# IanMadlenya/pyconsensus

Hardware: AMD Instinct MI355X
Metric: oracle rounds/sec (batched 50x20, 1 GPU) (higher is better)
Workload: dtype f64; 1 GPU; C3: 65536 independent 50x20 oracle rounds per GPU per step (one wavefront per round), inputs resident in HBM, every output of the result dict written (original and filled included); rounds_per_gpu=65536, reporters=50, events=20, parallelism=rounds sharded across 1 GPU(s), no collective

## Files before the change

### pyconsensus_amd/csrc/pcx_batched.hip

```cpp
#include <hip/hip_runtime.h>
#include <stdint.h>
#include <stdlib.h>

#include "pcx_internal.h"

namespace pcx {

namespace {

constexpr int W = 64;
constexpr int NMAX = 64;
constexpr int EMAX = 32;
static_assert(EMAX <= 2 * 16, "2 x 2 grid of 16 x 16 MFMA tiles");
static_assert(NMAX == W, "one reporter per lane");
constexpr int PACKED_WAVES = 4;

constexpr double PI_TOL = 1e-14;
constexpr int PI_MAXIT = 256;
constexpr int PI_PRESQUARE = 3;
constexpr int PI_SQUARE_EVERY = 32;
constexpr int PI_MAX_SQUARINGS = 8;
constexpr int PI_POLISH = 2;
constexpr double DBL_MIN_ = 2.2250738585072014e-308;
constexpr double DBL_EPS = 2.220446049250313080847e-16;

__device__ __forceinline__ int lane_id() { return threadIdx.x; }

#define PCX_OUTLINE __forceinline__

#define STAMP(k)                                                                  \
    do {                                                                          \
        if (a.stamps) {                                                           \
            const long long t_ = (long long)__builtin_amdgcn_s_memtime();         \
            if (threadIdx.x == 0) a.stamps[b * 32 + (k)] = t_;                    \
        }                                                                         \
    } while (0)

__device__ __forceinline__ void wsync() {
    __builtin_amdgcn_fence(__ATOMIC_RELEASE, "wavefront");
    __builtin_amdgcn_wave_barrier();
    __builtin_amdgcn_fence(__ATOMIC_ACQUIRE, "wavefront");
}

__device__ __forceinline__ uint64_t ballot(bool p) { return __ballot(p); }

__device__ __forceinline__ int popc(uint64_t m) { return __popcll(m); }

__device__ __forceinline__ double bcast(double v, int src) {
    const uint64_t u = (uint64_t)__double_as_longlong(v);
    const uint32_t lo = (uint32_t)__builtin_amdgcn_readlane((int)(uint32_t)u, src);
    const uint32_t hi = (uint32_t)__builtin_amdgcn_readlane((int)(uint32_t)(u >> 32), src);
    return __longlong_as_double((long long)(((uint64_t)hi << 32) | lo));
}

template <int CTRL>
__device__ __forceinline__ uint32_t dpp32(uint32_t v) {
    return (uint32_t)__builtin_amdgcn_update_dpp(0, (int)v, CTRL, 0xf, 0xf, false);
}
template <int S>
__device__ __forceinline__ uint32_t xor_lane32(uint32_t v) {
    if constexpr (S == 1) return dpp32<0xB1>(v);
    else if constexpr (S == 2) return dpp32<0x4E>(v);
    else if constexpr (S == 8) return dpp32<0x128>(v);
    else {
        static_assert(S == 4, "row-local distances only");
        const uint32_t up = dpp32<0x114>(v), dn = dpp32<0x104>(v);
        return (threadIdx.x & 4) ? up : dn;
    }
}

template <int S>
__device__ __forceinline__ double xor_lane(double v) {
    const uint64_t u = (uint64_t)__double_as_longlong(v);
    const uint32_t lo = xor_lane32<S>((uint32_t)u), hi = xor_lane32<S>((uint32_t)(u >> 32));
    return __longlong_as_double((long long)(((uint64_t)hi << 32) | lo));
}

__device__ __forceinline__ double lane_value(double v, int k) {
    const uint64_t u = (uint64_t)__double_as_longlong(v);
    const uint32_t lo = (uint32_t)__builtin_amdgcn_readlane((int)(uint32_t)u, k);
    const uint32_t hi = (uint32_t)__builtin_amdgcn_readlane((int)(uint32_t)(u >> 32), k);
    return __longlong_as_double((long long)(((uint64_t)hi << 32) | lo));
}

template <int ROWS = 4>
__device__ __forceinline__ double tree_sum(double v) {
    static_assert(ROWS == 1 || ROWS == 2 || ROWS == 4, "live 16-lane rows");
    v = v + xor_lane<1>(v);
    v = v + xor_lane<2>(v);
    v = v + xor_lane<4>(v);
    v = v + xor_lane<8>(v);
    if constexpr (ROWS == 1) return lane_value(v, 0);
    if constexpr (ROWS == 2) return lane_value(v, 0) + lane_value(v, 16);
    return (lane_value(v, 0) + lane_value(v, 16)) + (lane_value(v, 32) + lane_value(v, 48));
}
constexpr int live_rows(int ET) { return ET > 0 ? (ET <= 16 ? 1 : ET <= 32 ? 2 : 4) : 4; }

template <int D>
__device__ __forceinline__ double shr_lane(double v) {
    const uint64_t u = (uint64_t)__double_as_longlong(v);
    const uint32_t lo = (uint32_t)__builtin_amdgcn_update_dpp(0, (int)(uint32_t)u, 0x110 + D, 0xf, 0xf, false);
    const uint32_t hi = (uint32_t)__builtin_amdgcn_update_dpp(0, (int)(uint32_t)(u >> 32), 0x110 + D, 0xf, 0xf, false);
    return __longlong_as_double((long long)(((uint64_t)hi << 32) | lo));
}
__device__ __forceinline__ double wave_scan_d(double v) {
    v = v + shr_lane<1>(v);
    v = v + shr_lane<2>(v);
    v = v + shr_lane<4>(v);
    v = v + shr_lane<8>(v);
    const double r0 = lane_value(v, 15), r1 = lane_value(v, 31), r2 = lane_value(v, 47);
    const int row = threadIdx.x >> 4;
    const double r01 = r0 + r1;
    return row == 0 ? v : v + (row == 1 ? r0 : row == 2 ? r01 : r01 + r2);
}

template <int ROWS = 4>
__device__ __forceinline__ double wave_max(double v) {
    static_assert(ROWS == 1 || ROWS == 2 || ROWS == 4, "live 16-lane rows");
    v = fmax(v, xor_lane<1>(v));
    v = fmax(v, xor_lane<2>(v));
    v = fmax(v, xor_lane<4>(v));
    v = fmax(v, xor_lane<8>(v));
    if constexpr (ROWS == 1) return lane_value(v, 0);
    if constexpr (ROWS == 2) return fmax(lane_value(v, 0), lane_value(v, 16));
    return fmax(fmax(lane_value(v, 0), lane_value(v, 16)), fmax(lane_value(v, 32), lane_value(v, 48)));
}

__device__ __forceinline__ double catch_(double x, double tol) {
    if (x < 1.5 - tol) return 1.0;
    if (x > 1.5 + tol) return 2.0;
    return 1.5;
}

__device__ __forceinline__ double readlane_d(double v, int k) {
    const uint64_t u = (uint64_t)__double_as_longlong(v);
    const uint32_t lo = (uint32_t)__builtin_amdgcn_readlane((int)(uint32_t)u, k);
    const uint32_t hi = (uint32_t)__builtin_amdgcn_readlane((int)(uint32_t)(u >> 32), k);
    return __longlong_as_double((long long)(((uint64_t)hi << 32) | lo));
}

__device__ __forceinline__ double shr1_d(double v) {
    const uint64_t u = (uint64_t)__double_as_longlong(v);
    const uint32_t lo = (uint32_t)__builtin_amdgcn_update_dpp(0, (int)(uint32_t)u, 0x138, 0xf, 0xf, true);
    const uint32_t hi = (uint32_t)__builtin_amdgcn_update_dpp(0, (int)(uint32_t)(u >> 32), 0x138, 0xf, 0xf, true);
    return __longlong_as_double((long long)(((uint64_t)hi << 32) | lo));
}

__device__ __forceinline__ double permute_d(int dst_lane, double v) {
    const uint64_t u = (uint64_t)__double_as_longlong(v);
    const uint32_t lo = (uint32_t)__builtin_amdgcn_ds_permute(dst_lane * 4, (int)(uint32_t)u);
    const uint32_t hi = (uint32_t)__builtin_amdgcn_ds_permute(dst_lane * 4, (int)(uint32_t)(u >> 32));
    return __longlong_as_double((long long)(((uint64_t)hi << 32) | lo));
}

__device__ __forceinline__ double bpermute_d(int src_lane, double v) {
    const uint64_t u = (uint64_t)__double_as_longlong(v);
    const uint32_t lo = (uint32_t)__builtin_amdgcn_ds_bpermute(src_lane * 4, (int)(uint32_t)u);
    const uint32_t hi = (uint32_t)__builtin_amdgcn_ds_bpermute(src_lane * 4, (int)(uint32_t)(u >> 32));
    return __longlong_as_double((long long)(((uint64_t)hi << 32) | lo));
}

__device__ __forceinline__ int mbcnt64(uint64_t m) {
    return __builtin_amdgcn_mbcnt_hi((uint32_t)(m >> 32), __builtin_amdgcn_mbcnt_lo((uint32_t)m, 0));
}

__device__ PCX_OUTLINE double wave_pw_sum(double v, bool sel) {
    const int l = lane_id();
    const uint64_t m = ballot(sel);
    const int n = popc(m);
    if (n < 8) {
        double res = 0.0;
        uint64_t mm = m;
        while (mm) {
            const int k = __builtin_ctzll(mm);
            mm &= mm - 1;
            res += readlane_d(v, k);
        }
        return res;
    }
    const int p = sel ? mbcnt64(m) : n + mbcnt64(~m);
    const double a = permute_d((p & 7) * 8 + (p >> 3), v);
    const int T = n >> 3;
    double c = a;
    for (int t = 1; t < T; t++) {
        const double prev = shr1_d(c);
        c = (l & 7) == 0 ? a : prev + a;
    }
    const double r0 = readlane_d(c, 0 * 8 + T - 1), r1 = readlane_d(c, 1 * 8 + T - 1);
    const double r2 = readlane_d(c, 2 * 8 + T - 1), r3 = readlane_d(c, 3 * 8 + T - 1);
    const double r4 = readlane_d(c, 4 * 8 + T - 1), r5 = readlane_d(c, 5 * 8 + T - 1);
    const double r6 = readlane_d(c, 6 * 8 + T - 1), r7 = readlane_d(c, 7 * 8 + T - 1);
    double res = ((r0 + r1) + (r2 + r3)) + ((r4 + r5) + (r6 + r7));
    for (int q = 8 * T; q < n; q++) res += readlane_d(a, (q & 7) * 8 + (q >> 3));
    return res;
}

template <int NC>
__device__ PCX_OUTLINE double wave_pw_sum_prefix(double v, int nrt) {
    const int l = lane_id();
    const int n = NC > 0 ? NC : nrt;
    if (n < 8) {
        double res = 0.0;
        for (int k = 0; k < n; k++) res += readlane_d(v, k);
        return res;
    }
    const double a = permute_d((l & 7) * 8 + (l >> 3), v);
    const int T = n >> 3;
    double c = a;
    for (int t = 1; t < T; t++) {
        const double prev = shr1_d(c);
        c = (l & 7) == 0 ? a : prev + a;
    }
    const double r0 = readlane_d(c, 0 * 8 + T - 1), r1 = readlane_d(c, 1 * 8 + T - 1);
    const double r2 = readlane_d(c, 2 * 8 + T - 1), r3 = readlane_d(c, 3 * 8 + T - 1);
    const double r4 = readlane_d(c, 4 * 8 + T - 1), r5 = readlane_d(c, 5 * 8 + T - 1);
    const double r6 = readlane_d(c, 6 * 8 + T - 1), r7 = readlane_d(c, 7 * 8 + T - 1);
    double res = ((r0 + r1) + (r2 + r3)) + ((r4 + r5) + (r6 + r7));
    for (int q = 8 * T; q < n; q++) res += readlane_d(a, (q & 7) * 8 + (q >> 3));
    return res;
}

template <int D>
__device__ __forceinline__ double shl_lane(double v) {
    const uint64_t u = (uint64_t)__double_as_longlong(v);
    const uint32_t lo = dpp32<0x100 + D>((uint32_t)u), hi = dpp32<0x100 + D>((uint32_t)(u >> 32));
    return __longlong_as_double((long long)(((uint64_t)hi << 32) | lo));
}

__device__ __forceinline__ double pw_tree8(double c) {
    c = c + xor_lane<1>(c);
    c = c + xor_lane<2>(c);
    return c + shl_lane<4>(c);
}

template <int NC>
__device__ PCX_OUTLINE double wave_pw_sum_lds(double v, int nrt, double* scr) {
    const int l = lane_id();
    const int n = NC > 0 ? NC : nrt;
    if (n < 8) {
        double res = 0.0;
        for (int k = 0; k < n; k++) res += readlane_d(v, k);
        return res;
    }
    wsync();
    if (l < n) scr[l] = v;
    wsync();
    const int T = n >> 3;
    const double* const p = scr + (l & 7);
    double c = p[0];
    if constexpr (NC > 0) {
#pragma unroll
        for (int t = 1; t < NC / 8; t++) c = c + p[8 * t];
    } else {
        for (int t = 1; t < T; t++) c = c + p[8 * t];
    }
    c = pw_tree8(c);
    for (int q = 8 * T; q < n; q++) c = c + scr[q];
    return readlane_d(c, 0);
}

template <int NC>
__device__ PCX_OUTLINE void wave_pw_sum2_lds(double v1, double v2, int nrt, double* scr, double& s1, double& s2) {
    const int l = lane_id();
    const int n = NC > 0 ? NC : nrt;
    if (n < 8) {
        double r1 = 0.0, r2 = 0.0;
        for (int k = 0; k < n; k++) {
            r1 += readlane_d(v1, k);
            r2 += readlane_d(v2, k);
        }
        s1 = r1;
        s2 = r2;
        return;
    }
    wsync();
    if (l < n) {
        scr[l] = v1;
        scr[n + l] = v2;
    }
    wsync();
    const int T = n >> 3;
    const double* const base = scr + ((l & 8) ? n : 0);
    const double* const p = base + (l & 7);
    double c = p[0];
    if constexpr (NC > 0) {
#pragma unroll
        for (int t = 1; t < NC / 8; t++) c = c + p[8 * t];
    } else {
        for (int t = 1; t < T; t++) c = c + p[8 * t];
    }
    c = pw_tree8(c);
    for (int q = 8 * T; q < n; q++) c = c + base[q];
    s1 = readlane_d(c, 0);
    s2 = readlane_d(c, 8);
}

template <int NC>
__device__ PCX_OUTLINE double wave_pw_sum_dpp(double v, int nrt) {
    const int n = NC > 0 ? NC : nrt;
    if (n < 8 || n >= 24) return wave_pw_sum_prefix<NC>(v, nrt);
    const int T = n >> 3;
    double c = v;
    if (T == 2) c = v + shl_lane<8>(v);
    c = pw_tree8(c);
    double res = readlane_d(c, 0);
    for (int q = 8 * T; q < n; q++) res += readlane_d(v, q);
    return res;
}

__device__ __forceinline__ double dot2(const double* a, const double* b, int bs, int n) {
    double s = 0.0, c = 0.0;
    for (int i = 0; i < n; i++) {
        const double x = a[i], y = b[i * bs];
        const double p = x * y;
        const double pe = fma(x, y, -p);
        const double t = s + p;
        const double z = t - s;
        const double se = (s - (t - z)) + (p - z);
        s = t;
        c = c + (pe + se);
    }
    return s + c;
}

__device__ __noinline__ double ob_ddot(const double* v, const double* f, int ld, int n) {
    double acc8[4][8], acc4[4][4];
#pragma unroll
    for (int r = 0; r < 4; r++)
#pragma unroll
        for (int q = 0; q < 8; q++) acc8[r][q] = 0.0;
    const int n32 = n & -32, n16 = n & -16;
    for (int i = 0; i < n32; i += 32)
#pragma unroll
        for (int k = 0; k < 32; k++) acc8[k / 8][k % 8] = fma(v[i + k], f[(i + k) * ld], acc8[k / 8][k % 8]);
#pragma unroll
    for (int r = 0; r < 4; r++)
#pragma unroll
        for (int q = 0; q < 4; q++) acc4[r][q] = acc8[r][q] + acc8[r][q + 4];
    for (int i = n32; i < n16; i += 16)
#pragma unroll
        for (int k = 0; k < 16; k++) acc4[k / 4][k % 4] = fma(v[i + k], f[(i + k) * ld], acc4[k / 4][k % 4]);
    double A[4];
#pragma unroll
    for (int q = 0; q < 4; q++) A[q] = ((acc4[0][q] + acc4[1][q]) + acc4[2][q]) + acc4[3][q];
    double d = (A[0] + A[2]) + (A[1] + A[3]);
    for (int i = n16; i < n; i++) d = fma(v[i], f[i * ld], d);
    return d;
}

__device__ PCX_OUTLINE double ob_vecmat(const double* v, const double* f, int ld, int N, int E, int j) {
    if (E == 1) return ob_ddot(v, f, ld, N);
    if (j < (E & ~3)) {
        double y = 0.0;
        int n = 0;
        for (; n + 4 <= N; n += 4) {
            double t = f[(n + 1) * ld] * v[n + 1];
            t = fma(f[n * ld], v[n], t);
            t = fma(f[(n + 2) * ld], v[n + 2], t);
            t = fma(f[(n + 3) * ld], v[n + 3], t);
            y = y + t;
        }
        if (n + 2 <= N) {
            double t = f[(n + 1) * ld] * v[n + 1];
            t = fma(f[n * ld], v[n], t);
            y = y + t;
            n += 2;
        }
        if (n < N) y = y + f[n * ld] * v[n];
        return y;
    }
    double t = 0.0;
    int i = 0;
    if (E == 2 || E == 3)
        for (; i + 4 <= N; i += 4) {
            t = t + fma(f[i * ld], v[i], f[(i + 1) * ld] * v[i + 1]);
            t = t + fma(f[(i + 2) * ld], v[i + 2], f[(i + 3) * ld] * v[i + 3]);
        }
    for (; i < N; i++) t = fma(f[i * ld], v[i], t);
    return t;
// ... 274 lines not shown


__device__ __forceinline__ void round_to_global(double* dst, const double* F, int N, int E, int ES, int NT, int ET) {
    const int l = lane_id();
    if (NT > 0 && ET > 0 && (NT * ET) % 2 == 0 && ((uintptr_t)dst & 15) == 0) {
        const int tot2 = NT * ET / 2;
        for (int q = l; q < tot2; q += W) {
            const int idx = 2 * q;
            const int i0 = idx / ET, j0 = idx - i0 * ET;
            const int i1 = (idx + 1) / ET, j1 = idx + 1 - i1 * ET;
            reinterpret_cast<double2*>(dst)[q] = double2{F[i0 * ES + j0], F[i1 * ES + j1]};
        }
    } else {
        for (int idx = l; idx < N * E; idx += W) {
            const int i = idx / E, j = idx - i * E;
            dst[idx] = F[i * ES + j];
        }
    }
}

__device__ PCX_OUTLINE double rank_avg(const double* v, int E) {
    const int l = lane_id();
    double r = 0.0;
    if (l < E) {
        const double x = v[l];
        int lt = 0, eq = 0;
        for (int k = 0; k < E; k++) {
            const double y = v[k];
            lt += y < x;
            eq += y == x;
        }
        r = (double)lt + (double)(eq + 1) * 0.5;
        if (__builtin_isnan(x)) r = __builtin_nan("");
    }
    return r;
}

__device__ PCX_OUTLINE void rank_avg3(const double* v0, const double* v1, const double* v2, int E, double& r0,
                                      double& r1, double& r2) {
    const int l = lane_id();
    const int g = (l >= E) + (l >= 2 * E);
    const double* v = g == 0 ? v0 : g == 1 ? v1 : v2;
    double r = 0.0;
    if (l < 3 * E) {
        const double x = v[l - g * E];
        int lt = 0, eq = 0;
        for (int k = 0; k < E; k++) {
            const double y = v[k];
            lt += y < x;
            eq += y == x;
        }
        r = (double)lt + (double)(eq + 1) * 0.5;
        if (__builtin_isnan(x)) r = __builtin_nan("");
    }
    r0 = r;
    r1 = bpermute_d(l + E, r);
    r2 = bpermute_d(l + 2 * E, r);
}

struct Smem {
    double* F;
    double* C;
    double* M;
    double* rep;
    double* n1;
    double* n2;
    double* smooth;
    double* mu;
    double* tot;
    double* guess;
    double* x;
    double* ld;
    double* old;
    double* nv1;
    double* nv2;
    double* adj;
    uint64_t* miss;
};

__host__ __device__ inline int smem_rows(int N) { return (N + 1) & ~1; }
__host__ __device__ inline int cert_stride(int N, int ES) { return (ES & 1) ? (N | 1) : N; }
__host__ __device__ inline int smem_f_size(int N, int E, int ES) {
    return N * ES > E * cert_stride(N, ES) ? N * ES : E * cert_stride(N, ES);
}
__host__ __device__ inline int smem_evs(int E) { return (E + 1) & ~1; }
__host__ __device__ inline int smem_mat(int E, int ES, bool pk) { return pk ? E * (E + 1) / 2 : E * ES; }
__host__ __device__ inline int smem_c_size(int N, int E, int ES, bool pk) {
    if (pk) return smem_rows(N) + 2 * smem_evs(E);
    const int need = 3 * smem_rows(N) + 2 * smem_evs(E);
    return smem_mat(E, ES, pk) > need ? smem_mat(E, ES, pk) : need;
}
__host__ __device__ inline int smem_m_size(int N, int E, int ES, int NR, bool pk) {
    const int scr = med_scr(NR) + smem_evs(E);
    if (pk) {
        const int vec = 2 * smem_rows(N) + 2 * smem_evs(E);
        const int rest = smem_mat(E, ES, pk) - smem_c_size(N, E, ES, pk);
        const int need = scr > vec ? scr : vec;
        return need > rest ? need : rest;
    }
    const int need = scr > 2 * smem_evs(E) ? scr : 2 * smem_evs(E);
    return smem_mat(E, ES, pk) > need ? smem_mat(E, ES, pk) : need;
}

__host__ __device__ inline size_t smem_doubles(int N, int E, int ES, int NR, bool pk) {
    return (size_t)smem_f_size(N, E, ES) + smem_c_size(N, E, ES, pk) + smem_m_size(N, E, ES, NR, pk) +
           (pk ? 1 : 4) * (size_t)smem_evs(E);
}

template <bool PK>
__device__ __forceinline__ int sym_at(int j, int k, int ES) {
    if constexpr (PK)
        return j >= k ? j * (j + 1) / 2 + k : k * (k + 1) / 2 + j;
    else
        return j * ES + k;
}

__device__ Smem carve(double* base, int N, int E, int ES, int NR, bool pk) {
    const int nr = smem_rows(N), ne = smem_evs(E);
    Smem s;
    double* p = base;
    s.F = p; p += smem_f_size(N, E, ES);
    s.C = p; p += smem_c_size(N, E, ES, pk);
    s.M = p; p += smem_m_size(N, E, ES, NR, pk);
    s.miss = reinterpret_cast<uint64_t*>(p); p += ne;
    s.mu = s.x = s.ld = nullptr;
    if (!pk) {
        s.mu = p; p += ne;
        s.x = p; p += ne;
        s.ld = p; p += ne;
    }
    s.tot = s.M + med_scr(NR);
    s.rep = s.C + ne;
    s.guess = s.C;
    if (pk) {
        s.smooth = s.C;
        s.adj = s.C + nr;
        s.old = s.C + nr + ne;
        s.n1 = s.M;
        s.n2 = s.M + nr;
        s.nv1 = s.M + 2 * nr;
        s.nv2 = s.M + 2 * nr + ne;
    } else {
        s.n1 = s.C;
        s.n2 = s.C + nr;
        s.smooth = s.C + 2 * nr;
        s.adj = s.C + 3 * nr;
        s.old = s.C + 3 * nr + ne;
        s.nv1 = s.M;
        s.nv2 = s.M + ne;
    }
    return s;
}

template <bool PK, int ROWS = 4>
__device__ PCX_OUTLINE double matvec_unit(const double* M, int ES, double xv, int E) {
    const int l = lane_id(), r = l < E ? l : 0;
    double acc = 0.0;
    for (int k = 0; k < E; k++) acc = fma(M[sym_at<PK>(r, k, ES)], lane_value(xv, k), acc);
    const double y = l < E ? acc : 0.0;
    const double nrm = sqrt(tree_sum<ROWS>(l < E ? y * y : 0.0));
    return l < E ? y / nrm : 0.0;
}

typedef double d4v __attribute__((ext_vector_type(4)));

__device__ __forceinline__ d4v mfma_f64(double a, double b, d4v c) {
    return __builtin_amdgcn_mfma_f64_16x16x4f64(a, b, c, 0, 0, 0);
}

template <bool PK>
__device__ PCX_OUTLINE void square_scaled(double* M, int ES, int E) {
    const int l = lane_id(), ml = l & 15, kq = l >> 4;
    const bool two = E > 16;
    d4v t00 = {0, 0, 0, 0}, t01 = {0, 0, 0, 0}, t10 = {0, 0, 0, 0}, t11 = {0, 0, 0, 0};
    for (int m0 = 0; m0 < E; m0 += 4) {
        const int mm = m0 + kq;
        const bool ok = mm < E;
        const double a0 = (ok && ml < E) ? M[sym_at<PK>(ml, mm, ES)] : 0.0;
        const double b0 = a0;
        t00 = mfma_f64(a0, b0, t00);
        if (two) {
            const double a1 = (ok && 16 + ml < E) ? M[sym_at<PK>(16 + ml, mm, ES)] : 0.0;
            const double b1 = a1;
            if (!PK) t01 = mfma_f64(a0, b1, t01);
            t10 = mfma_f64(a1, b0, t10);
            t11 = mfma_f64(a1, b1, t11);
        }
    }
    double mx = 0.0;
#pragma unroll
    for (int r = 0; r < 4; r++) {
        const int j0 = kq + 4 * r, j1 = 16 + kq + 4 * r, k0 = ml, k1 = 16 + ml;
        if (j0 < E && k0 < E) mx = fmax(mx, fabs(t00[r]));
        if (!PK && j0 < E && k1 < E) mx = fmax(mx, fabs(t01[r]));
        if (j1 < E && k0 < E) mx = fmax(mx, fabs(t10[r]));
        if (j1 < E && k1 < E) mx = fmax(mx, fabs(t11[r]));
    }
    mx = wave_max(mx);
    const bool pow2 = mx >= DBL_MIN_ && __builtin_isfinite(mx);
    const double sc = pow2 ? ldexp(1.0, -ilogb(mx)) : 1.0;
    auto scaled = [&](double t) { return pow2 ? t * sc : (mx > 0.0 ? t / mx : t); };
    wsync();
#pragma unroll
    for (int r = 0; r < 4; r++) {
        const int j0 = kq + 4 * r, j1 = 16 + kq + 4 * r, k0 = ml, k1 = 16 + ml;
        if (j0 < E && k0 < E && (!PK || k0 <= j0)) M[sym_at<PK>(j0, k0, ES)] = scaled(t00[r]);
        if (j0 < E && k1 < E && !PK) M[sym_at<PK>(j0, k1, ES)] = scaled(t01[r]);
        if (j1 < E && k0 < E) M[sym_at<PK>(j1, k0, ES)] = scaled(t10[r]);
        if (j1 < E && k1 < E && (!PK || k1 <= j1)) M[sym_at<PK>(j1, k1, ES)] = scaled(t11[r]);
    }
    wsync();
}

template <int NS>
struct SymOps {
    double a0[NS], a1[NS];
};

template <int NS>
__device__ __forceinline__ void load_sym_ops(const double* C, int E, SymOps<NS>& m) {
    const int l = lane_id(), ml = l & 15, kq = l >> 4;
    const bool two = E > 16;
#pragma unroll
    for (int s = 0; s < NS; s++) {
        m.a0[s] = 0.0;
        m.a1[s] = 0.0;
        if (4 * s < E) {
            const int mm = 4 * s + kq;
            const bool ok = mm < E;
            if (ok && ml < E) m.a0[s] = C[sym_at<true>(ml, mm, 0)];
            if (two && ok && 16 + ml < E) m.a1[s] = C[sym_at<true>(16 + ml, mm, 0)];
        }
    }
}

template <int NS>
__device__ __forceinline__ void store_sym_ops(double* C, int E, const SymOps<NS>& m) {
    const int l = lane_id(), ml = l & 15, kq = l >> 4;
    const bool two = E > 16;
    wsync();
#pragma unroll
    for (int s = 0; s < NS; s++) {
        if (4 * s < E) {
            const int mm = 4 * s + kq;
            if (mm <= ml && ml < E) C[sym_at<true>(ml, mm, 0)] = m.a0[s];
            if (two && mm <= 16 + ml && 16 + ml < E) C[sym_at<true>(16 + ml, mm, 0)] = m.a1[s];
        }
    }
    wsync();
}

template <int NS>
__device__ PCX_OUTLINE void square_scaled_reg(SymOps<NS>& m, int E) {
    const int l = lane_id(), ml = l & 15, kq = l >> 4;
    const bool two = E > 16;
    const bool t01_moves = E <= 20;
    d4v t00 = {0, 0, 0, 0}, t01 = {0, 0, 0, 0}, t10 = {0, 0, 0, 0}, t11 = {0, 0, 0, 0};
#pragma unroll
    for (int s = 0; s < NS; s++) {
        if (4 * s < E) {
            t00 = mfma_f64(m.a0[s], m.a0[s], t00);
            if (two) {
                if (!t01_moves) t01 = mfma_f64(m.a0[s], m.a1[s], t01);
                t10 = mfma_f64(m.a1[s], m.a0[s], t10);
                t11 = mfma_f64(m.a1[s], m.a1[s], t11);
            }
        }
    }
    double mx = 0.0;
#pragma unroll
    for (int r = 0; r < 4; r++) {
        const int j0 = kq + 4 * r, j1 = 16 + kq + 4 * r, k0 = ml, k1 = 16 + ml;
        if (j0 < E && k0 < E) mx = fmax(mx, fabs(t00[r]));
        if (j1 < E && k0 < E) mx = fmax(mx, fabs(t10[r]));
        if (j1 < E && k1 < E) mx = fmax(mx, fabs(t11[r]));
    }
    mx = wave_max(mx);
    const bool pow2 = mx >= DBL_MIN_ && __builtin_isfinite(mx);
    const double sc = pow2 ? ldexp(1.0, -ilogb(mx)) : 1.0;
    auto keep = [&](auto scaled) {
#pragma unroll
        for (int r = 0; r < 4; r++) {
            const int j0 = kq + 4 * r, j1 = 16 + kq + 4 * r, k0 = ml, k1 = 16 + ml;
            if (r < NS) m.a0[r] = (j0 < E && k0 < E) ? scaled(t00[r]) : 0.0;
            if (two) {
                if (r < NS) {
                    if (t01_moves) {
                        const double s10 = (16 + kq < E && k0 < E) ? scaled(t10[0]) : 0.0;
                        const double v = bpermute_d(16 * (ml & 3) + 4 * r + kq, s10);
                        m.a1[r] = (j0 < E && k1 < E) ? v : 0.0;
                    } else {
                        m.a1[r] = (j0 < E && k1 < E) ? scaled(t01[r]) : 0.0;
                    }
                }
                if (4 + r < NS) {
                    m.a0[4 + r] = (j1 < E && k0 < E) ? scaled(t10[r]) : 0.0;
                    m.a1[4 + r] = (j1 < E && k1 < E) ? scaled(t11[r]) : 0.0;
                }
            }
        }
    };
    if (pow2)
        keep([&](double t) { return t * sc; });
    else
        keep([&](double t) { return mx > 0.0 ? t / mx : t; });
}

constexpr int JAC_MAXSWEEP = 30;
constexpr double JAC_TOL = 1e-15;

__device__ __forceinline__ void jac_pair(int i, int r, int n, int& p, int& q) {
// ... 523 lines not shown
```

### pyconsensus_amd/csrc/pcx_batched_round.inc

```
#if PCX_ROUND_RAGGED >= 2
#define PCX_ROUND_CELL0 rcell
#define PCX_ROUND_ROW0 rrow
#define PCX_ROUND_EV0 rev
#define PCX_ROUND_B rround
template <int NT, int ET, bool CLUS, bool PK>
#if PCX_ROUND_RAGGED == 3
__global__ void __launch_bounds__(64, 3) ragged_kmeans_round_kernel(BatchArgs ka, const MediumDesc* __restrict__ rag,
                                                                    const RoundParams* __restrict__ ptab,
                                                                    const KmeansEntry* __restrict__ ktab) {
#else
__global__ void __launch_bounds__(64, 3) ragged_params_round_kernel(BatchArgs ka, const MediumDesc* __restrict__ rag,
                                                                    const RoundParams* __restrict__ ptab) {
#endif
    static_assert(NT == 0 && ET == 0, "a ragged launch has no compiled shape");
    extern __shared__ __attribute__((aligned(16))) double smem[];
    const MediumDesc* const rd = rag + blockIdx.x;
    const int N = __builtin_amdgcn_readfirstlane(rd->N), E = __builtin_amdgcn_readfirstlane(rd->E), ES = E | 1;
    const int64_t rcell = uniform64(rd->cell), rrow = uniform64(rd->row), rev = uniform64(rd->ev);
    const int64_t rround = __builtin_amdgcn_readfirstlane(rd->round);
    const RoundParams* const rp = ptab + __builtin_amdgcn_readfirstlane(rd->param);
    BatchArgs a = ka;
    a.algorithm = __builtin_amdgcn_readfirstlane(rp->algorithm);
    a.max_components = __builtin_amdgcn_readfirstlane(rp->max_components);
    a.catch_tol = uniform_f64(rp->catch_tol);
// ... 259 lines not shown
#pragma unroll 10
                for (int i = 0; i < NR; i++) {
                    if (i < N) {
                        const double t = (S.rep[i] / tot) * Fc[i * ES];
                        ex = ((miss_j >> i) & 1) ? ex : ex + t;
                    }
                }
                if ((need_bin >> l) & 1) {
                    double gs = catch_(ex, a.catch_tol);
                    if (a.int_dtype) gs = trunc(gs);
                    S.guess[l] = gs;
                }
            }
            if (col && miss_j) S.tot[l] = tot;
            wsync();
        }
        while (todo) {
            const int j = __builtin_ctzll(todo);
            todo &= todo - 1;
            double x0, w0;
            bool p0;
            pair_of(j, x0, w0, p0);
            finish(j, wave_wmedian_rank<(NT > 0 ? NT : 64)>(x0, w0, p0, N, S.M, a.stamps ? mprof : nullptr));
            wsync();
        }
    }
    wsync();
    STAMP(14);
    if (row) {
        uint64_t mn = S.miss[0];
        double gn = S.guess[0];
        for (int j = 0; j < E; j++) {
            const uint64_t mj = mn;
            const double g = gn;
            if (j + 1 < E) {
                mn = S.miss[j + 1];
                gn = S.guess[j + 1];
            }
            if ((mj >> l) & 1) S.F[l * ES + j] = g;
        }
    }
    wsync();
    if (double* const fg = out_args()->filled) round_to_global(fg + PCX_ROUND_CELL0, S.F, N, E, ES, NT, ET);

    STAMP(3);
    double oldj = col ? ob_vecmat(S.rep, S.F + l, ES, N, E, l) : 0.0;

    double sc_i = 0.0, nc_i = 0.0, ld_j = 0.0;
    int branch = 5, flags = 0, iters = 0, comps = -1;
    const int alg = a.algorithm;
    const bool clus = CLUS && alg >= 5;
    const double rep_sum = pw_rows(rep);
    if (alg == 0 || alg == 2 || alg == 3 || clus) {
        const double den = rep_sum;
        double muj = 0.0;
        if (E == 1) {
            const double p = row ? S.F[l * ES] * rep : 0.0;
            const double acc = pw_rows(p);
            muj = acc / den;
        } else if (col) {
            double acc = S.F[l] * S.rep[0];
            for (int i = 1; i < N; i++) acc = acc + S.F[i * ES + l] * S.rep[i];
            muj = acc / den;
        }
        if constexpr (!PK) {
            wsync();
            if (col) S.mu[l] = muj;
            wsync();
        }

        STAMP(4);
        bool nonzero = false, finite = true;
        {
            constexpr int NR = NT > 0 ? NT : 64;
            const int ml = l & 15, kq = l >> 4;
            const bool two = E > 16;
            const double m0 = __shfl(muj, ml), m1 = __shfl(muj, 16 + ml);
            const double mu0 = ml < E ? m0 : 0.0, mu1 = 16 + ml < E ? m1 : 0.0;
            d4v c00 = {0, 0, 0, 0}, c10 = {0, 0, 0, 0}, c11 = {0, 0, 0, 0};
#pragma unroll
            for (int i0 = 0; i0 < NR; i0 += 4) {
                if (i0 < N) {
                    const int i = i0 + kq;
                    const bool ok = i < N;
                    const double tk = ok ? trunc(S.rep[i] * 1e6) : 0.0;
                    const bool v0 = ok && ml < E, v1 = ok && 16 + ml < E;
                    const double d0 = v0 ? S.F[i * ES + ml] - mu0 : 0.0;
                    const double d1 = v1 ? S.F[i * ES + 16 + ml] - mu1 : 0.0;
                    const double a0 = v0 ? d0 * tk : 0.0, a1 = v1 ? d1 * tk : 0.0;
                    c00 = mfma_f64(a0, d0, c00);
                    if (two) {
                        c10 = mfma_f64(a1, d0, c10);
                        c11 = mfma_f64(a1, d1, c11);
                    }
                }
            }
            auto put = [&](int j, int k, double acc) {
                const double c = acc / denom;
                S.C[sym_at<PK>(j, k, ES)] = c;
                if (!PK) {
                    S.M[sym_at<PK>(j, k, ES)] = c;
                    S.C[k * ES + j] = c;
                    S.M[k * ES + j] = c;
                }
                nonzero |= c != 0.0;
                finite &= __builtin_isfinite(c) != 0;
            };
            if constexpr (PK) wsync();
#pragma unroll
            for (int r = 0; r < 4; r++) {
                const int j0 = kq + 4 * r, j1 = 16 + kq + 4 * r, k0 = ml, k1 = 16 + ml;
                if (j0 < E && k0 <= j0) put(j0, k0, c00[r]);
                if (j1 < E && k0 < E) put(j1, k0, c10[r]);
                if (j1 < E && k1 <= j1) put(j1, k1, c11[r]);
            }
        }
        const bool any_nz = ballot(nonzero) != 0;
        const bool all_fin = ballot(!finite) == 0;
        wsync();

        STAMP(5);
        double xv = 0.0;
        if (!all_fin) {
            xv = col ? 1.0 : 0.0;
            flags |= 2;
        } else if (!any_nz) {
            xv = l == 0 ? 1.0 : 0.0;
            flags |= 1;
        } else {
            const double dg = col ? S.C[sym_at<PK>(l, l, ES)] : -__builtin_inf();
            const double dgmax = wave_max<CR>(dg);
            const int kd = __builtin_ctzll(ballot(col && dg == dgmax));
            double x0 = col ? S.C[sym_at<PK>(l, kd, ES)] : 0.0;
            const double n0 = sqrt(tree_sum<CR>(x0 * x0));
            xv = col ? x0 / n0 : 0.0;
            constexpr int NS = !PK ? 1 : ET > 0 ? (ET + 3) / 4 : EMAX / 4;
            SymOps<NS> mreg, creg;
            if constexpr (PK) {
                load_sym_ops<NS>(S.C, E, mreg);
                creg = mreg;
            }
            auto square = [&](bool in_loop) {
                if constexpr (PK) {
                    if (in_loop) load_sym_ops<NS>(S.C, E, mreg);
                    square_scaled_reg<NS>(mreg, E);
                    if (in_loop) store_sym_ops<NS>(S.C, E, mreg);
                } else {
                    square_scaled<PK>(S.M, ES, E);
                }
            };
            int sqn = 0;
            for (; sqn < PI_PRESQUARE; sqn++) square(false);
            if constexpr (PK) store_sym_ops<NS>(S.C, E, mreg);
            int it = 0, since = 0;
            for (;;) {
                const double y = matvec_unit<PK, CR>(PK ? S.C : S.M, ES, xv, E);
                const bool moved = ballot(col && fabs(y - xv) > PI_TOL) != 0;
                xv = y;
                it++;
                since++;
                if (!moved) break;
                if (it >= PI_MAXIT) {
                    flags |= 4;
                    break;
                }
                if (since >= PI_SQUARE_EVERY && sqn < PI_MAX_SQUARINGS) {
                    square(true);
                    sqn++;
                    since = 0;
                }
            }
            if constexpr (PK) store_sym_ops<NS>(S.C, E, creg);
            for (int p = 0; p < PI_POLISH; p++) xv = matvec_unit<PK, CR>(S.C, ES, xv, E);
            const uint64_t nzm = ballot(col && xv != 0.0);
            if (nzm) {
                const double xf = bcast(xv, __builtin_ctzll(nzm));
                const bool neg = popc(nzm) == 1 ? xf < 0.0 : xf > 0.0;
                if (neg) xv = -xv;
            }
            iters = it + PI_POLISH + sqn;
        }
        const double nv = sqrt(pw_cols(xv * xv));
        ld_j = col ? xv / nv : 0.0;
        wsync();
        if (clus) {
        } else if (alg == 0) {
            const int r = row ? l : 0;
            double acc = 0.0;
            for (int j = 0; j < E; j++) acc = fma(S.F[r * ES + j] - lane_value(muj, j), lane_value(ld_j, j), acc);
            if (row) sc_i = acc;
        } else if (flags & 2) {
            sc_i = __builtin_nan("");
        } else if constexpr (!PK) {
            const double trace = pw_cols(col ? S.C[l * ES + l] : 0.0);
            wsync();
            for (int o = l; o < E * E; o += W) {
                const int j = o / E, k = o - j * E;
                S.M[j * ES + k] = S.C[j * ES + k];
            }
            wsync();
            jacobi_eig_wave(S.M, S.C, ES, E, S.x, S.ld);
            const double sig = col ? fabs(S.M[l * ES + l]) : 0.0;
            if (col) S.nv1[l] = sig;
            wsync();
            if (col) {
                int rk = 0;
                for (int k = 0; k < E; k++) rk += (S.nv1[k] > sig) | ((S.nv1[k] == sig) & (k < l));
                S.nv2[rk] = (double)l;
            }
            wsync();
#if PCX_ROUND_RAGGED
            const int kmax = alg == 2 && a.max_components < E ? a.max_components : E;
#else
            const int kmax = alg == 2 ? a.max_components : E;
#endif
            double net = 0.0, ve = 0.0;
            int used = kmax;
            for (int c = 0; c < kmax; c++) {
                const int idx = (int)S.nv2[c];
                const double sg = S.nv1[idx];
                const double fl = S.C[idx] < 0.0 ? -1.0 : 1.0;
                if (row) {
                    double d = 0.0;
                    for (int j = 0; j < E; j++) d = fma(S.F[l * ES + j] - S.mu[j], fl * S.C[j * ES + idx], d);
                    net = net + sg * d;
                }
                if (alg == 3) {
                    ve = ve + sg / trace;
                    if (ve >= a.variance_threshold) {
                        used = c + 1;
                        break;
                    }
                }
            }
            comps = alg == 3 ? used : -1;
            sc_i = net;
            wsync();
        }
    } else if (alg == 4) {
        sc_i = row ? a.aux_scores[PCX_ROUND_ROW0 + l] : 0.0;
    }
    STAMP(6);
    if constexpr (CLUS) {
        if (clus) {
            double* X = smem + smem_doubles(N, E, ES, NRM, PK);
            if (alg == 6)
                nc_i = hier_nc(S.F, S.mu, ES, N, E, a.hierarchy_threshold, reinterpret_cast<uint64_t*>(X));
#if !PCX_ROUND_RAGGED
            else if (alg == 5)
                nc_i = kmeans_nc(a, b, S.F, S.mu, ES, N, E, X);
#elif PCX_ROUND_RAGGED == 3
            else if (alg == 5)
                nc_i = kmeans_nc(a, 0, S.F, S.mu, ES, N, E, X);
#endif
            else
                nc_i = feck_nc(a, S.F, ES, N, E, rep, X);
            wsync();
        }
    }
    if (alg != 1 && !clus) {
        const bool any_nan = ballot(row && __builtin_isnan(sc_i)) != 0;
        double mn = wave_max(row ? -sc_i : -__builtin_inf());
        mn = -mn;
        double mx = wave_max(row ? sc_i : -__builtin_inf());
        if (any_nan) {
            mn = __builtin_nan("");
            mx = __builtin_nan("");
        }
        const double set1 = sc_i + fabs(mn);
        const double set2 = sc_i - mx;
        double a1 = fabs(set1), a2 = fabs(set2);
        double S1, S2;
        pw_rows2(a1, a2, S1, S2);
        if (S1 == 0) {
            a1 += 1.0;
            S1 = pw_rows(a1);
        }
        if (S2 == 0) {
            a2 += 1.0;
            S2 = pw_rows(a2);
        }
        if (row) {
            S.n1[l] = a1 / S1;
            S.n2[l] = a2 / S2;
        }
        if (col) S.old[l] = oldj;
        wsync();
        double d1 = 0.0, d2 = 0.0;
        {
            const int jc = l & 31;
            double d = 0.0;
            if (jc < E) d = ob_vecmat(l < 32 ? S.n1 : S.n2, S.F + jc, ES, N, E, jc);
            const uint64_t du = (uint64_t)__double_as_longlong(d);
            const int up = ((l + 32) & 63) << 2;
            const uint32_t ulo = (uint32_t)__builtin_amdgcn_ds_bpermute(up, (int)(uint32_t)du);
            const uint32_t uhi = (uint32_t)__builtin_amdgcn_ds_bpermute(up, (int)(uint32_t)(du >> 32));
            if (col) {
                d1 = d;
                d2 = __longlong_as_double((long long)(((uint64_t)uhi << 32) | ulo));
            }
        }
        if (col) {
            const double t = 0.01 * oldj;
            S.nv1[l] = d1 + t;
            S.nv2[l] = d2 + t;
        }
        wsync();
        double ref = 0.0;
        if (alg == 0) {
            double r0, r1, r2;
            if (3 * E <= W) {
                rank_avg3(S.old, S.nv1, S.nv2, E, r0, r1, r2);
            } else {
                r0 = rank_avg(S.old, E);
                r1 = rank_avg(S.nv1, E);
                r2 = rank_avg(S.nv2, E);
            }
            const double e1 = fabs(r1 - r0), e2 = fabs(r2 - r0);
            ref = pw_cols(e1) - pw_cols(e2);
        }
        bool pick1;
        if (ref == 0) {
            const double q1 = d1 - oldj, q2 = d2 - oldj;
            const double ref2 = pw_cols(q1 * q1) - pw_cols(q2 * q2);
            pick1 = ref2 <= 0;
            branch = pick1 ? 3 : 4;
        } else {
            pick1 = ref < 0;
            branch = pick1 ? 1 : 2;
        }
        nc_i = pick1 ? set1 : set2;
    }

    STAMP(7);
    const double meanrep = rep_sum / (double)N;
    double u = fabs(nc_i * (rep / meanrep));
    double Su = pw_rows(u);
    const bool rep_masked = alg == 0 && __builtin_isnan(Su);
    if (Su == 0) {
        u += 1.0;
        Su = pw_rows(u);
    }
// ... 248 lines not shown
```

Before: 70.98 million rounds/s.

## Use DPP row-broadcast FMAs and permlane swaps for power-iteration matvec and scores

Replaces the per-column readlane broadcasts in the power-iteration matvec and the PCA score loop with permlane16/32 swaps that spread the vector across rows. These feed inline-asm v_fmac_f64_dpp row_newbcast instructions, so each column term becomes a single DPP FMA instead of scalar readlanes followed by an FMA. The column loop is fully unrolled at compile time per event count, and packed-triangle LDS addresses are precomputed. The DPP helpers now set bound_ctrl, and the xor-4 step in tree_sum and wave_max becomes a shift-left by 4. This adds hand-written asm with s_nop hazard padding and depends on gfx950 permlane swap builtins.

```diff
diff --git a/pyconsensus_amd/csrc/pcx_batched.hip b/pyconsensus_amd/csrc/pcx_batched.hip
--- a/pyconsensus_amd/csrc/pcx_batched.hip
+++ b/pyconsensus_amd/csrc/pcx_batched.hip
@@ -1,6 +1,8 @@
 #include <hip/hip_runtime.h>
 #include <stdint.h>
 #include <stdlib.h>
+
+#include <type_traits>
 
 #include "pcx_internal.h"
 
@@ -55,7 +57,7 @@
 
 template <int CTRL>
 __device__ __forceinline__ uint32_t dpp32(uint32_t v) {
-    return (uint32_t)__builtin_amdgcn_update_dpp(0, (int)v, CTRL, 0xf, 0xf, false);
+    return (uint32_t)__builtin_amdgcn_update_dpp(0, (int)v, CTRL, 0xf, 0xf, true);
 }
 template <int S>
 __device__ __forceinline__ uint32_t xor_lane32(uint32_t v) {
@@ -76,6 +78,13 @@
     return __longlong_as_double((long long)(((uint64_t)hi << 32) | lo));
 }
 
+template <int D>
+__device__ __forceinline__ double shl_lane(double v) {
+    const uint64_t u = (uint64_t)__double_as_longlong(v);
+    const uint32_t lo = dpp32<0x100 + D>((uint32_t)u), hi = dpp32<0x100 + D>((uint32_t)(u >> 32));
+    return __longlong_as_double((long long)(((uint64_t)hi << 32) | lo));
+}
+
 __device__ __forceinline__ double lane_value(double v, int k) {
     const uint64_t u = (uint64_t)__double_as_longlong(v);
     const uint32_t lo = (uint32_t)__builtin_amdgcn_readlane((int)(uint32_t)u, k);
@@ -88,7 +97,7 @@
     static_assert(ROWS == 1 || ROWS == 2 || ROWS == 4, "live 16-lane rows");
     v = v + xor_lane<1>(v);
     v = v + xor_lane<2>(v);
-    v = v + xor_lane<4>(v);
+    v = v + shl_lane<4>(v);
     v = v + xor_lane<8>(v);
     if constexpr (ROWS == 1) return lane_value(v, 0);
     if constexpr (ROWS == 2) return lane_value(v, 0) + lane_value(v, 16);
@@ -99,8 +108,8 @@
 template <int D>
 __device__ __forceinline__ double shr_lane(double v) {
     const uint64_t u = (uint64_t)__double_as_longlong(v);
-    const uint32_t lo = (uint32_t)__builtin_amdgcn_update_dpp(0, (int)(uint32_t)u, 0x110 + D, 0xf, 0xf, false);
-    const uint32_t hi = (uint32_t)__builtin_amdgcn_update_dpp(0, (int)(uint32_t)(u >> 32), 0x110 + D, 0xf, 0xf, false);
+    const uint32_t lo = (uint32_t)__builtin_amdgcn_update_dpp(0, (int)(uint32_t)u, 0x110 + D, 0xf, 0xf, true);
+    const uint32_t hi = (uint32_t)__builtin_amdgcn_update_dpp(0, (int)(uint32_t)(u >> 32), 0x110 + D, 0xf, 0xf, true);
     return __longlong_as_double((long long)(((uint64_t)hi << 32) | lo));
 }
 __device__ __forceinline__ double wave_scan_d(double v) {
@@ -119,7 +128,7 @@
     static_assert(ROWS == 1 || ROWS == 2 || ROWS == 4, "live 16-lane rows");
     v = fmax(v, xor_lane<1>(v));
     v = fmax(v, xor_lane<2>(v));
-    v = fmax(v, xor_lane<4>(v));
+    v = fmax(v, shl_lane<4>(v));
     v = fmax(v, xor_lane<8>(v));
     if constexpr (ROWS == 1) return lane_value(v, 0);
     if constexpr (ROWS == 2) return fmax(lane_value(v, 0), lane_value(v, 16));
@@ -218,13 +227,6 @@
     double res = ((r0 + r1) + (r2 + r3)) + ((r4 + r5) + (r6 + r7));
     for (int q = 8 * T; q < n; q++) res += readlane_d(a, (q & 7) * 8 + (q >> 3));
     return res;
-}
-
-template <int D>
-__device__ __forceinline__ double shl_lane(double v) {
-    const uint64_t u = (uint64_t)__double_as_longlong(v);
-    const uint32_t lo = dpp32<0x100 + D>((uint32_t)u), hi = dpp32<0x100 + D>((uint32_t)(u >> 32));
-    return __longlong_as_double((long long)(((uint64_t)hi << 32) | lo));
 }
 
 __device__ __forceinline__ double pw_tree8(double c) {
@@ -805,11 +807,85 @@
     return s;
 }
 
-template <bool PK, int ROWS = 4>
-__device__ PCX_OUTLINE double matvec_unit(const double* M, int ES, double xv, int E) {
+struct RowSpread {
+    double lo, hi;
+};
+__device__ __forceinline__ double pack_d(uint32_t lo, uint32_t hi) {
+    return __longlong_as_double((long long)(((uint64_t)hi << 32) | lo));
+}
+__device__ __forceinline__ void dpp_ready(RowSpread& s) { asm("s_nop 1" : "+v"(s.lo), "+v"(s.hi)); }
+__device__ __forceinline__ RowSpread row_spread2(double v) {
+    const uint64_t u = (uint64_t)__double_as_longlong(v);
+    const auto a = __builtin_amdgcn_permlane16_swap((uint32_t)u, (uint32_t)u, false, false);
+    const auto b = __builtin_amdgcn_permlane16_swap((uint32_t)(u >> 32), (uint32_t)(u >> 32), false, false);
+    RowSpread s = {pack_d(a[0], b[0]), pack_d(a[1], b[1])};
+    dpp_ready(s);
+    return s;
+}
+__device__ __forceinline__ RowSpread row_spread4(double v) {
+    const uint64_t u = (uint64_t)__double_as_longlong(v);
+    const auto a = __builtin_amdgcn_permlane16_swap((uint32_t)u, (uint32_t)u, false, false);
+    const auto b = __builtin_amdgcn_permlane16_swap((uint32_t)(u >> 32), (uint32_t)(u >> 32), false, false);
+    const uint32_t ll = __builtin_amdgcn_permlane32_swap(a[0], a[0], false, false)[0];
+    const uint32_t lh = __builtin_amdgcn_permlane32_swap(b[0], b[0], false, false)[0];
+    const uint32_t hl = __builtin_amdgcn_permlane32_swap(a[1], a[1], false, false)[0];
+    const uint32_t hh = __builtin_amdgcn_permlane32_swap(b[1], b[1], false, false)[0];
+    RowSpread s = {pack_d(ll, lh), pack_d(hl, hh)};
+    dpp_ready(s);
+    return s;
+}
+template <int K, bool NEG = false>
+__device__ __forceinline__ void fmac_rowbcast(double& acc, const RowSpread& s, double m) {
+    static_assert(K >= 0 && K < 32, "a column of a two-row vector");
+    if constexpr (NEG)
+        asm("v_fmac_f64_dpp %0, -%1, %2 row_newbcast:%3 row_mask:0xf bank_mask:0xf"
+            : "+v"(acc)
+            : "v"(K < 16 ? s.lo : s.hi), "v"(m), "n"(K & 15));
+    else
+        asm("v_fmac_f64_dpp %0, %1, %2 row_newbcast:%3 row_mask:0xf bank_mask:0xf"
+            : "+v"(acc)
+            : "v"(K < 16 ? s.lo : s.hi), "v"(m), "n"(K & 15));
+}
+template <int K>
+__device__ __forceinline__ double sub_rowbcast(double f, const RowSpread& s, double one) {
+    fmac_rowbcast<K, true>(f, s, one);
+    return f;
+}
+template <int K, int ET, class F>
+__device__ __forceinline__ void static_cols(F&& f) {
+    if constexpr (K < ET) {
+        f(std::integral_constant<int, K>());
+        static_cols<K + 1, ET>(f);
+    }
+}
+
+typedef const __attribute__((address_space(3))) double* LdsDoubles;
+struct SymBase {
+    uint32_t tri, row;
+};
+__device__ __forceinline__ SymBase sym_base(const double* M, int r) {
+    const uint32_t m = (uint32_t)(uintptr_t)(LdsDoubles)M;
+    SymBase b = {m + (uint32_t)(r * (r + 1) / 2 * 8), m + (uint32_t)(r * 8)};
+    asm("" : "+v"(b.tri), "+v"(b.row));
+    return b;
+}
+template <bool PK, int K>
+__device__ __forceinline__ double sym_col(const double* M, const SymBase& b, int r, int ES) {
+    if constexpr (!PK) return M[r * ES + K];
+    const uint32_t at = K <= r ? b.tri : b.row + 8u * (K * (K + 1) / 2 - K);
+    return ((LdsDoubles)(uintptr_t)at)[K];
+}
+
+template <bool PK, int ROWS = 4, int ET = 0>
+__device__ PCX_OUTLINE double matvec_unit(const double* M, int ES, double xv, int E, const SymBase& sb) {
     const int l = lane_id(), r = l < E ? l : 0;
     double acc = 0.0;
-    for (int k = 0; k < E; k++) acc = fma(M[sym_at<PK>(r, k, ES)], lane_value(xv, k), acc);
+    if constexpr (ET > 0 && ET <= 32) {
+        const RowSpread x = row_spread2(xv);
+        static_cols<0, ET>([&](auto k) { fmac_rowbcast<k.value>(acc, x, sym_col<PK, k.value>(M, sb, r, ES)); });
+    } else {
+        for (int k = 0; k < E; k++) acc = fma(M[sym_at<PK>(r, k, ES)], lane_value(xv, k), acc);
+    }
     const double y = l < E ? acc : 0.0;
     const double nrm = sqrt(tree_sum<ROWS>(l < E ? y * y : 0.0));
     return l < E ? y / nrm : 0.0;
diff --git a/pyconsensus_amd/csrc/pcx_batched_round.inc b/pyconsensus_amd/csrc/pcx_batched_round.inc
--- a/pyconsensus_amd/csrc/pcx_batched_round.inc
+++ b/pyconsensus_amd/csrc/pcx_batched_round.inc
@@ -435,9 +435,10 @@
             int sqn = 0;
             for (; sqn < PI_PRESQUARE; sqn++) square(false);
             if constexpr (PK) store_sym_ops<NS>(S.C, E, mreg);
+            const SymBase sb = sym_base(S.C, col ? l : 0);
             int it = 0, since = 0;
             for (;;) {
-                const double y = matvec_unit<PK, CR>(PK ? S.C : S.M, ES, xv, E);
+                const double y = matvec_unit<PK, CR, ET>(PK ? S.C : S.M, ES, xv, E, sb);
                 const bool moved = ballot(col && fabs(y - xv) > PI_TOL) != 0;
                 xv = y;
                 it++;
@@ -454,7 +455,7 @@
                 }
             }
             if constexpr (PK) store_sym_ops<NS>(S.C, E, creg);
-            for (int p = 0; p < PI_POLISH; p++) xv = matvec_unit<PK, CR>(S.C, ES, xv, E);
+            for (int p = 0; p < PI_POLISH; p++) xv = matvec_unit<PK, CR, ET>(S.C, ES, xv, E, sb);
             const uint64_t nzm = ballot(col && xv != 0.0);
             if (nzm) {
                 const double xf = bcast(xv, __builtin_ctzll(nzm));
@@ -470,7 +471,16 @@
         } else if (alg == 0) {
             const int r = row ? l : 0;
             double acc = 0.0;
-            for (int j = 0; j < E; j++) acc = fma(S.F[r * ES + j] - lane_value(muj, j), lane_value(ld_j, j), acc);
+            if constexpr (ET > 0 && ET <= 32) {
+                const RowSpread mu = row_spread4(muj), ld = row_spread4(ld_j);
+                double one = 1.0;
+                asm("s_nop 1" : "+v"(one));
+                static_cols<0, ET>([&](auto j) {
+                    fmac_rowbcast<j.value>(acc, ld, sub_rowbcast<j.value>(S.F[r * ES + j.value], mu, one));
+                });
+            } else {
+                for (int j = 0; j < E; j++) acc = fma(S.F[r * ES + j] - lane_value(muj, j), lane_value(ld_j, j), acc);
+            }
             if (row) sc_i = acc;
         } else if (flags & 2) {
             sc_i = __builtin_nan("");
```

After: 73.45 million rounds/s (median of 6 runs). 1.03x the previous value.
